# hezy18/SegMMInterest

Measured on AMD Instinct MI355X. Metric: train interactions/sec (segment-Transformer, B=512·S=40·D=768), higher is better.
Workload: dtype f32 (products via scaled fp16x2 split, 22-bit operands, fp32 accumulate; operands pre-split by their producers); 1 GPU; BASELINE config 2: synthetic SegMM B=512/GPU x S=40 x D_in=768 -> d=768, h=16, 2-layer segment encoder, image/image inputs, Lt=100 user tokens, interestBPR, dropout 0.1, AdamW; 8 distinct batches rotated; input=features; rows_per_gpu=512, global_batch=512, segments=40, feat_dim=768, in_dim=768, layers=2, parallelism=dp1, grad_allreduce_overlap=True, input_prefetch=False, delayed_scale_overflows=0, gemm_engine=f16x3p

## Files before the change

segmminterest_amd/csrc/capi.hip:

```cpp
#include <stdarg.h>
#include <stdio.h>
#include <string.h>
#include <stdlib.h>
#include <initializer_list>
#include <type_traits>

#include "../../include/segmm_hip.h"
#include "attention16.h"
#include "attention_pl.h"
#include "attention_stream.h"
#include "attention_wide.h"
#include "common.h"
#include "evalops.h"
#include "gemm.h"
#include "gemm_split.h"
#include "gemm_planes.h"
#include "gemm_planes8.h"
#include "gemm_planes4.h"
#include "loss.h"
#include "rowops.h"
#include "assemble.h"
#include "storeops.h"
#include "srops.h"

static int num_cus() {
    static int n = 0;
    if (n == 0) {
        int dev = 0;
        hipDeviceProp_t prop;
        if (hipGetDevice(&dev) == hipSuccess && hipGetDeviceProperties(&prop, dev) == hipSuccess) n = prop.multiProcessorCount;
        if (n <= 0) n = 256;
    }
    return n;
}
#ifdef SEGMM_STAMPS
static unsigned long long* g_segmm_stamps = nullptr;
extern "C" int segmm_debug_set_stamps(void* p) { g_segmm_stamps = (unsigned long long*)p; return 0; }
#endif

thread_local char g_segmm_err[512] = {0};

int segmm_fail(int code, const char* fmt, ...) {
    va_list ap;
    va_start(ap, fmt);
    vsnprintf(g_segmm_err, sizeof(g_segmm_err), fmt, ap);
    va_end(ap);
    return code;
}

#define LAUNCH_CHECK() SEGMM_CHECK_HIP(hipGetLastError())

StepState* g_segmm_step = nullptr;
static StepState* g_step_default = nullptr;
StepState* segmm_step_current() {
    if (g_segmm_step) return g_segmm_step;
    if (!g_step_default) {
        if (hipMalloc((void**)&g_step_default, sizeof(StepState)) != hipSuccess) return nullptr;
        (void)hipMemset(g_step_default, 0, sizeof(StepState));
    }
    return g_step_default;
}

using namespace segmm;

static inline int attn_keys_p(int La, int Lb) { return ((La + 15) & ~15) + ((Lb + 15) & ~15); }
static int attn_fill(AttnArgs& a, int B, int H, int dh, int Lq, int La, int Lb, const float* Qa, const float* Qb, int ldq,
                     const float* Ka, const float* Va, int ldka, const float* Kb, const float* Vb, int ldkb,
                     const uint8_t* mq, const uint8_t* mka, const uint8_t* mkb, float drop_p, uint64_t seed,
                     uint32_t site, bool planes_in = false) {
    SEGMM_REQUIRE(B > 0 && H > 0 && Lq > 0 && La >= 0 && Lb >= 0 && La + Lb > 0, "attn: empty dimension");
    if (La == 0) { Qa = Qb; Ka = Kb; Va = Vb; ldka = ldkb; mka = mkb; }
    if (Lb == 0) { Qb = Qa; Kb = Ka; Vb = Va; ldkb = ldka; mkb = mka; }
    SEGMM_REQUIRE(((Qa && Qb && Ka && Va && Kb && Vb) || (planes_in && !Qa && !Qb && !Ka && !Va && !Kb && !Vb)) && mq && mka && mkb, "attn: null pointer");
    SEGMM_REQUIRE(dh == 4 || dh == 8 || dh == 16 || dh == 32 || dh == 48 || dh == 64 || dh == 96 || dh == 128,
                  "attn: head dim %d not built (4,8,16,32,48,64,96,128)", dh);
    SEGMM_REQUIRE(!(planes_in && att_wide(dh)), "attn: input planes are not built for wide heads (head dim %d > 64): hand the fp32 views of Q / K / V", dh);
    SEGMM_REQUIRE(ldq % 4 == 0 && ldka % 4 == 0 && ldkb % 4 == 0, "attn: leading dims %% 4");
    SEGMM_REQUIRE(aligned16(Qa) && aligned16(Qb) && aligned16(Ka) && aligned16(Va) && aligned16(Kb) && aligned16(Vb), "attn: alignment");
    SEGMM_REQUIRE(Lq <= 256 && La <= 256 && Lb <= 256, "attn: Lq=%d, La=%d, Lb=%d not built (at most 256 queries and 256 keys per key block)", Lq, La, Lb);
    a.B = B; a.H = H; a.Lq = Lq; a.La = La; a.Lb = Lb;
    a.Qa = Qa; a.Qb = Qb; a.ldq = ldq; a.Ka = Ka; a.Va = Va; a.ldka = ldka; a.Kb = Kb; a.Vb = Vb; a.ldkb = ldkb;
    a.mq = mq; a.mka = mka; a.mkb = mkb;
    a.scale = 1.0f / sqrtf((float)dh);
    a.drop = make_drop(drop_p, seed, site);
    {
        const size_t ka = La ? ((size_t)B * La - 1) * ldka + (size_t)H * dh : 0, kb = Lb ? ((size_t)B * Lb - 1) * ldkb + (size_t)H * dh : 0;
        const size_t q = ((size_t)B * Lq - 1) * ldq + (size_t)H * dh;
        SEGMM_REQUIRE(((size_t)B * La + 16) * ldka * 4 < (1ull << 32) && ((size_t)B * Lb + 16) * ldkb * 4 < (1ull << 32) &&
                      ((size_t)B * Lq + 16) * ldq * 4 < (1ull << 32), "attn: a K/V/Q view exceeds the 4 GiB buffer-addressing window");
        a.ka_bytes = (uint32_t)(ka * 4); a.kb_bytes = (uint32_t)(kb * 4); a.q_bytes = (uint32_t)(q * 4);
    }
    return 0;
}

enum {
    K_ATTN, K_ATT_FWD_PL, K_ATT_FWD_LDS, K_ATT_FWD_KSPLIT, K_ATT_FWD_LDS_PAD, K_ATT_STREAM, K_ATT_FUSED_LAUNCH, K_ATT_MERGE, K_ATT_LDS_PAD, K_ATT_WAVES, K_ATT_WAVES_PL, K_ATT_REPAIR_WALK,
    K_ATT_HPB_FWD, K_ATT_HPB_DQ, K_ATT_HPB_DKV, K_L1NORM_REG, K_GEMM_BN, K_PL_VAR, K_PL_NJ, K_TN_VAR, K_LN_BWD_PARTS, K_DPRE_PLANES_ONLY, K_EMA_NT, K_LN_FWD_PARTS, K_COUNT
};
struct Knob { const char* name; int value; const char* doc; };
static Knob g_knobs[K_COUNT] = {
    {"ATTN", 1, "attention arithmetic: 0 (env: f32) exact-fp32 kernels only, 1 fp16x3 where measured faster, 2 (env: f16all) fp16x3 wherever built"},
    {"ATT_FWD_PL", 1, "planes-in forward when the caller hands input planes (0: never)"},
    {"ATT_FWD_LDS", 1, "LDS-DMA staged fp32 forward: 0 never, 1 heads with >= 4 query tiles, 2 wherever it fits"},
    {"ATT_FWD_KSPLIT", 1, "staged forward: key-tile groups per query tile"},
    {"ATT_FWD_LDS_PAD", 0, "probe: extra LDS bytes per forward workgroup (fewer workgroups per CU)"},
    {"ATT_STREAM", 0, "1: every fp32-view forward and every phase 0-3 backward through the streamed kernels (always taken above 192 padded keys)"},
    {"ATT_FUSED_LAUNCH", 2, "fused backward: 2 one launch per key block, 1 one launch for both"},
    {"ATT_MERGE", 1, "short heads: one workgroup per head for both key blocks in the fused backward"},
    {"ATT_LDS_PAD", 0, "probe: extra LDS bytes per backward workgroup"},
    {"ATT_WAVES", 4, "fused fp16x3 backward: waves per workgroup (key tiles in passes)"},
    {"ATT_WAVES_PL", 3, "planes-in fused backward: waves per workgroup, 1..4 (3: 40.7 KB of LDS -> four workgroups per CU for a 100-key block too)"},
    {"ATT_REPAIR_WALK", 512, "planes-in backward, repair launch: workgroups that walk the heads (0: one workgroup per head)"},
    {"ATT_HPB_FWD", 0, "forward workgroup shape heads | tiles << 8 (env: \"heads[,tiles]\"; 0: built-in)"},
    {"ATT_HPB_DQ", 0, "dQ kernel workgroup shape, as above"},
    {"ATT_HPB_DKV", 0, "dK/dV kernel workgroup shape, as above"},
    {"L1NORM_REG", 1, "L1 normalisation with the row held in registers"},
    {"GEMM_BN", 0, "on-the-fly GEMM: tile width override (0: built-in choice)"},
    {"PL_VAR", 4, "plane NT GEMM: 4 gemm_pl_nt4 (round 6: 128 x 256 tiles, two workgroups per CU) for K >= 768 and N >= 768, gemm_pl_nt8 otherwise; 44 gemm_pl_nt4 always; 8 gemm_pl_nt8 (round 3); 1: the round-2 fallback kernel for every launch"},
    {"PL_NJ", 0, "plane NT GEMM: tile width in 64-column units (0: modelled choice)"},
    {"TN_VAR", 8, "plane TN GEMM: 8 gemm_pl_tn4 (round 6: 128 x 256 tiles, two workgroups per CU) for few-tile and 128-row matrices, gemm_pl_tn8 (round 3) otherwise; 4 gemm_pl_tn4 wherever it fits; 88 gemm_pl_tn8 wherever it fits; 0: the round-2 fallback kernel for every launch"},
    {"LN_BWD_PARTS", 0, "LayerNorm backward: most workgroups (= partial rows of its column sums) per launch; 0: as many four-wave workgroups as are resident at the row width (768 at d = 768: one full round, no under-occupied tail)"},
    {"DPRE_PLANES_ONLY", 1, "embedding LayerNorm gradients as planes only + repair launch (no fp32 copy): 0 never, 1 for sites on the per-position grid today (rows * d >= 2^23), 2 wherever segmm_layernorm_bwd_pos_parts gives a grid (tests at small shapes), 3 as 1 for the user side only (A/B per site)"},
    {"EMA_NT", 0, "segmm_ema_update: 0 everything with the default cache policy, 1 the shadow loaded and stored nontemporally (p with the default policy); same bits (A/B: profiles/ema/)"},
    {"LN_FWD_PARTS", 0, "LayerNorm forward (d <= 1024): 0 one round of resident workgroups whose waves walk rows, grid by row width; 1 the one-wave-per-row form; 2 and up: that many workgroups in the walking form, clamped to 64..4096; same bits (A/B: profiles/row_stream/)"},
};
static bool g_knobs_ready = false;
static void knobs_init() {
    if (g_knobs_ready) return;
    g_knobs_ready = true;
    for (int k = 0; k < K_COUNT; ++k) {
        char name[64];
        snprintf(name, sizeof(name), "SEGMM_%s", g_knobs[k].name);
        const char* e = getenv(name);
        if (!e || !*e) continue;
        if (k == K_ATTN) g_knobs[k].value = !strcmp(e, "f32") ? 0 : !strcmp(e, "f16all") ? 2 : 1;
        else if (k == K_ATT_HPB_FWD || k == K_ATT_HPB_DQ || k == K_ATT_HPB_DKV) {
            const char* c = strchr(e, ',');
            g_knobs[k].value = (atoi(e) > 0 ? atoi(e) : 0) | ((c && atoi(c + 1) > 0 ? atoi(c + 1) : 0) << 8);
        } else g_knobs[k].value = atoi(e);
    }
}
static inline int knob(int k) { knobs_init(); return g_knobs[k].value; }
int segmm_config_set(const char* name, int value) {
    knobs_init();
    for (int k = 0; k < K_COUNT; ++k)
        if (!strcmp(name, g_knobs[k].name)) { const int prev = g_knobs[k].value; g_knobs[k].value = value; return prev; }
    return segmm_fail(-1, "segmm_config_set: no knob named %s (see segmm_config_dump)", name);
}
int segmm_config_dump(char* buf, int n) {
    knobs_init();
    int need = 0;
    for (int k = 0; k < K_COUNT; ++k) {
        char line[320];
        const int m = snprintf(line, sizeof(line), "SEGMM_%s=%d  # %s\n", g_knobs[k].name, g_knobs[k].value, g_knobs[k].doc);
        if (buf && need + m < n) memcpy(buf + need, line, (size_t)m + 1);
        need += m;
    }
    return need;
}

static int attn_f16() { return knob(K_ATTN); }

static void attn_shape(int n, int H, int max_waves, int want_default, int kn, int& wq, int& hpb) {
    wq = n;
    if (n > 5) {
        wq = 4;
        for (int w = 5; w >= 3; --w)
            if (n % w == 0) { wq = w; break; }
    }
    if (wq > max_waves) wq = max_waves;
    hpb = 1;
    const int e = knob(kn);
    int want = want_default;
    if (e & 0xff) {
        want = e & 0xff;
        if ((e >> 8) > 0 && (e >> 8) <= n && (e >> 8) <= max_waves) wq = e >> 8;
    }
    for (int c = want; c >= 1; --c)
        if (H % c == 0 && c * wq <= max_waves) { hpb = c; break; }
}

static bool attn_streamed(int Tp) { return Tp > 16 * 12 || knob(K_ATT_STREAM) != 0; }
template <class F>
static void attn_by_key_tiles(int Tp, F launch) {
    if (Tp <= 64) launch(std::integral_constant<int, 4>{});
    else if (Tp <= 160) launch(std::integral_constant<int, 10>{});
    else launch(std::integral_constant<int, 12>{});
}
template <int MAXW, class F>
static void attn_by_waves(int nw, F launch) {
    if (nw <= 4) launch(std::integral_constant<int, 4>{});
    else if (MAXW <= 8 || nw <= 8) launch(std::integral_constant<int, 8>{});
    else if constexpr (MAXW > 8) launch(std::integral_constant<int, 12>{});
}

template <int DH>
static bool attn_fwd_pl_takes(const AttnArgs& a) {
    if constexpr (DH % 16 != 0 || att_wide(DH)) return false;
    else {
        if (knob(K_ATT_FWD_PL) == 0) return false;
        const int nqt = (a.Lq + 15) / 16, T = a.La + a.Lb;
        return a.in.Qa && a.La % 4 == 0 && a.Lb % 4 == 0 && nqt <= ATT_PL_MAXW && T <= 16 * 12 &&
               attn_fwd_pl_lds_bytes<DH>(a.La, a.Lb) <= 160 * 1024 && (((uintptr_t)a.mka | (uintptr_t)a.mkb) & 3u) == 0;
    }
}
template <int DH>
static int attn_launch_fwd_pl(AttnArgs& a, hipStream_t s) {
// ... 297 lines not shown
#pragma unroll
    for (int i = 0; i < 8; ++i)
#pragma unroll
        for (int j = 0; j < 4; ++j) t += acc[i][j].x + acc[i][j].y + acc[i][j].z + acc[i][j].w;
    if (t == 12345.678f) out[0] = t;
}
}

namespace segmm {
__global__ void step_set_kernel(StepState* st, uint32_t lo, uint32_t hi, int step, float b1, float b2) {
    st->seed_lo = lo; st->seed_hi = hi; st->step = step;
    st->bc1 = step > 0 ? (float)(1.0 - pow((double)b1, (double)step)) : 1.f;
    st->bc2_sqrt = step > 0 ? (float)sqrt(1.0 - pow((double)b2, (double)step)) : 1.f;
    st->lr = (float)segmm_lr_at(*st, step - 1);
}
__global__ void step_advance_kernel(StepState* st, float b1, float b2) {
    const int t = st->step + 1;
    st->step = t;
    const uint32_t lo = mix32(st->seed_lo + 0x9E3779B9u * (uint32_t)t);
    st->seed_hi = mix32(st->seed_hi ^ lo ^ 0x85EBCA6Bu) & 0x7fffffffu;
    st->seed_lo = lo;
    st->bc1 = (float)(1.0 - pow((double)b1, (double)t));
    st->bc2_sqrt = (float)sqrt(1.0 - pow((double)b2, (double)t));
    st->lr = (float)segmm_lr_at(*st, t - 1);
}
__global__ void step_advance_guarded_kernel(StepState* st, float b1, float b2) {
    const int t = st->step + 1;
    st->step = t;
    const uint32_t lo = mix32(st->seed_lo + 0x9E3779B9u * (uint32_t)t);
    st->seed_hi = mix32(st->seed_hi ^ lo ^ 0x85EBCA6Bu) & 0x7fffffffu;
    st->seed_lo = lo;
    const int ta = t - (int)st->skipped;
    st->bc1 = ta > 0 ? (float)(1.0 - pow((double)b1, (double)ta)) : 1.f;
    st->bc2_sqrt = ta > 0 ? (float)sqrt(1.0 - pow((double)b2, (double)ta)) : 1.f;
    st->lr = (float)segmm_lr_at(*st, t - 1);
    st->skip = 0u;
}
__global__ void step_set_skipped_kernel(StepState* st, uint32_t skipped) {
    st->skip = 0u;
    st->skipped = skipped;
}
__global__ void step_schedule_kernel(StepState* st, int kind, float base_lr, int warmup_steps, float start_factor, int decay_steps,
                                     float eta_min, float gamma, int step_size) {
    st->kind = kind; st->base_lr = base_lr; st->warmup_steps = warmup_steps; st->start_factor = start_factor;
    st->decay_steps = decay_steps; st->eta_min = eta_min; st->gamma = gamma; st->step_size = step_size;
    st->lr = (float)segmm_lr_at(*st, st->step - 1);
}
__global__ void step_base_lr_kernel(StepState* st, float base_lr) {
    st->base_lr = base_lr;
    st->lr = (float)segmm_lr_at(*st, st->step - 1);
}
}

template <class F> static void with_bools(F&& f) { f(); }
template <class F, class... Bs> static void with_bools(F&& f, bool b, Bs... bs) {
    if (b) with_bools([&](auto... cs) { f(std::true_type{}, cs...); }, bs...);
    else with_bools([&](auto... cs) { f(std::false_type{}, cs...); }, bs...);
}

extern "C" {

const char* segmm_last_error(void) { return g_segmm_err; }
int segmm_abi_version(void) { return SEGMM_ABI_VERSION; }
int segmm_attn_mode(int mode) { const int prev = attn_f16(); if (mode >= 0 && mode <= 2) g_knobs[K_ATTN].value = mode; return prev; }

static PlaneOut plane_out(uint16_t* planes, int ld2, float* hdr, const float* scale_in) {
    PlaneOut po;
    po.p = (_Float16*)planes; po.ld2 = ld2; po.hdr = hdr; po.scale_in = scale_in;
    return po;
}
#define PLANE_OUT_CHECK(what, cols)                                                                                          \
    SEGMM_REQUIRE(!planes || (hdr && (cols) % 32 == 0 && ld2 % 64 == 0 && ld2 >= 2 * (cols) && aligned16(planes)),             \
                  what ": plane output needs a header, cols %% 32, ld2 %% 64, 16-byte alignment")

int segmm_l1norm(const float* x, float* y, float* inv_scale, int64_t rows, int D, float* amax, uint16_t* planes, int ld2, float* hdr,
                 const float* scale_in, segmm_stream_t stream) {
    PLANE_OUT_CHECK("l1norm", D);
    SEGMM_REQUIRE(x && (y || inv_scale || (planes && scale_in)), "l1norm: null pointer");
    SEGMM_REQUIRE(D > 0 && D % 4 == 0 && aligned16(x) && (!y || aligned16(y)), "l1norm: D %% 4 / alignment (D=%d)", D);
    if (rows <= 0) return 0;
    const int wpb = 4;
    const int reg_form = knob(K_L1NORM_REG);
    const dim3 grid((unsigned)((rows + wpb - 1) / wpb)), block(64 * wpb);
#define L1R(V) hipLaunchKernelGGL((l1norm_reg_kernel<V>), grid, block, 0, (hipStream_t)stream, x, y, inv_scale, (long long)rows, D, amax, plane_out(planes, ld2, hdr, scale_in))
    if (reg_form && D <= 256) L1R(1);
    else if (reg_form && D <= 512) L1R(2);
    else if (reg_form && D <= 768) L1R(3);
    else if (reg_form && D <= 1024) L1R(4);
    else if (reg_form && D <= 1536) L1R(6);
    else if (reg_form && D <= 2048) L1R(8);
    else hipLaunchKernelGGL(l1norm_kernel, grid, block, 0, (hipStream_t)stream, x, y, inv_scale, (long long)rows, D, amax, plane_out(planes, ld2, hdr, scale_in));
#undef L1R
    LAUNCH_CHECK();
    return 0;
}

static inline bool aligned8(const void* p) { return (((uintptr_t)p) & 7u) == 0; }
#define ROW_H_LAUNCH(KERNEL, ...)                                                                                        \
    do {                                                                                                                 \
        if (elem == SEGMM_ELEM_F16) { ROW_H_LAUNCH_V(KERNEL, ELEM_F16, __VA_ARGS__); }                                   \
        else { ROW_H_LAUNCH_V(KERNEL, ELEM_BF16, __VA_ARGS__); }                                                         \
    } while (0)
#define ROW_H_LAUNCH_V(KERNEL, E, ...)                                                                                   \
    do {                                                                                                                 \
        if (D <= 256) hipLaunchKernelGGL((KERNEL<E, 1>), grid, block, 0, (hipStream_t)stream, __VA_ARGS__);              \
        else if (D <= 512) hipLaunchKernelGGL((KERNEL<E, 2>), grid, block, 0, (hipStream_t)stream, __VA_ARGS__);         \
        else if (D <= 768) hipLaunchKernelGGL((KERNEL<E, 3>), grid, block, 0, (hipStream_t)stream, __VA_ARGS__);         \
        else if (D <= 1024) hipLaunchKernelGGL((KERNEL<E, 4>), grid, block, 0, (hipStream_t)stream, __VA_ARGS__);        \
        else if (D <= 1536) hipLaunchKernelGGL((KERNEL<E, 6>), grid, block, 0, (hipStream_t)stream, __VA_ARGS__);        \
        else if (D <= 256 * ROW_MAXV) hipLaunchKernelGGL((KERNEL<E, 8>), grid, block, 0, (hipStream_t)stream, __VA_ARGS__); \
        else hipLaunchKernelGGL((KERNEL<E, 0>), grid, block, 0, (hipStream_t)stream, __VA_ARGS__);                       \
    } while (0)

int segmm_l1norm_h(const uint16_t* x, int elem, float* y, float* inv_scale, int64_t rows, int D, float* amax, uint16_t* planes, int ld2,
                   float* hdr, const float* scale_in, segmm_stream_t stream) {
    PLANE_OUT_CHECK("l1norm_h", D);
    SEGMM_REQUIRE(elem == SEGMM_ELEM_F16 || elem == SEGMM_ELEM_BF16, "l1norm_h: elem = %d (SEGMM_ELEM_F16 = 1, SEGMM_ELEM_BF16 = 2)", elem);
    SEGMM_REQUIRE(x && (y || inv_scale || (planes && scale_in)), "l1norm_h: null pointer");
    SEGMM_REQUIRE(D > 0 && D % 4 == 0 && aligned8(x) && (!y || aligned16(y)), "l1norm_h: D %% 4 / alignment (D=%d)", D);
    if (rows <= 0) return 0;
    const dim3 grid((unsigned)((rows + 3) / 4)), block(256);
    ROW_H_LAUNCH(l1norm_h_kernel, x, y, inv_scale, (long long)rows, D, amax, plane_out(planes, ld2, hdr, scale_in));
    LAUNCH_CHECK();
    return 0;
}

static inline bool aligned4(const void* p) { return (((uintptr_t)p) & 3u) == 0; }
static inline bool elem8(int elem) { return elem == SEGMM_ELEM_E4M3 || elem == SEGMM_ELEM_E5M2 || elem == SEGMM_ELEM_I8; }
#define ROW_B_LAUNCH(KERNEL, ...)                                                                                        \
    do {                                                                                                                 \
        if (elem == SEGMM_ELEM_E4M3) { ROW_H_LAUNCH_V(KERNEL, ELEM_E4M3, __VA_ARGS__); }                                 \
        else if (elem == SEGMM_ELEM_E5M2) { ROW_H_LAUNCH_V(KERNEL, ELEM_E5M2, __VA_ARGS__); }                            \
        else { ROW_H_LAUNCH_V(KERNEL, ELEM_I8, __VA_ARGS__); }                                                           \
    } while (0)

int segmm_l1norm_b(const uint8_t* x, int elem, float* y, float* inv_scale, int64_t rows, int D, float* amax, uint16_t* planes, int ld2,
                   float* hdr, const float* scale_in, segmm_stream_t stream) {
    PLANE_OUT_CHECK("l1norm_b", D);
    SEGMM_REQUIRE(elem8(elem), "l1norm_b: elem = %d (SEGMM_ELEM_E4M3 = 3, SEGMM_ELEM_E5M2 = 4, SEGMM_ELEM_I8 = 5)", elem);
    SEGMM_REQUIRE(x && (y || inv_scale || (planes && scale_in)), "l1norm_b: null pointer");
    SEGMM_REQUIRE(D > 0 && D % 4 == 0 && aligned4(x) && (!y || aligned16(y)), "l1norm_b: D %% 4 / alignment (D=%d)", D);
    if (rows <= 0) return 0;
    const dim3 grid((unsigned)((rows + 3) / 4)), block(256);
    ROW_B_LAUNCH(l1norm_b_kernel, x, y, inv_scale, (long long)rows, D, amax, plane_out(planes, ld2, hdr, scale_in));
    LAUNCH_CHECK();
    return 0;
}

int segmm_quantize_rows(const float* x, int64_t rows, int D, int elem, uint8_t* q, float* scale_out, segmm_stream_t stream) {
    SEGMM_REQUIRE(elem8(elem), "quantize_rows: elem = %d (SEGMM_ELEM_E4M3 = 3, SEGMM_ELEM_E5M2 = 4, SEGMM_ELEM_I8 = 5)", elem);
    SEGMM_REQUIRE(x && q && rows >= 0, "quantize_rows: null pointer / rows");
    SEGMM_REQUIRE(D > 0 && D % 4 == 0 && aligned16(x) && aligned4(q) && (!scale_out || aligned4(scale_out)),
                  "quantize_rows: D %% 4 / alignment (D=%d)", D);
    if (rows <= 0) return 0;
    const dim3 grid((unsigned)((rows + 3) / 4)), block(256);
    if (elem == SEGMM_ELEM_E4M3) hipLaunchKernelGGL((quantize_rows_kernel<ELEM_E4M3>), grid, block, 0, (hipStream_t)stream, x, (long long)rows, D, q, scale_out);
    else if (elem == SEGMM_ELEM_E5M2) hipLaunchKernelGGL((quantize_rows_kernel<ELEM_E5M2>), grid, block, 0, (hipStream_t)stream, x, (long long)rows, D, q, scale_out);
    else hipLaunchKernelGGL((quantize_rows_kernel<ELEM_I8>), grid, block, 0, (hipStream_t)stream, x, (long long)rows, D, q, scale_out);
    LAUNCH_CHECK();
    return 0;
}

static int gemm_impl(int layout, int M, int N, int K, const float* A, int lda, const float* B, int ldb, float* C, int ldc,
                     const float* bias, const float* row_scale, const float* residual, int ldr, int res_period,
                     int activation, float* aux, int ldaux, float drop_p, uint64_t seed, uint32_t site, int splits,
                     float* workspace, int accumulate, int engine, const uint16_t* a_planes, long long a_pstride,
                     const uint16_t* b_planes, long long b_pstride, int nplanes, const float* a_amax, int a_namax,
// ... 1941 lines not shown
```

segmminterest_amd/csrc/gemm_planes.h:

```cpp
#pragma once
#include <type_traits>
#include "gemm_split.h"

namespace segmm {

struct PlaneOperand {
    const _Float16* p; int ld2;
    uint32_t bytes;
    const float* hdr;
    const float* f32; int ldf;
};
struct PGemmX {
    PlaneOperand A, B;
    _Float16* Cp; int ldc2; float* c_hdr;
    const float* c_scale_in;
    int write_c;
    int repair;
    float* colsum_out; float* colsum_ws;
    int dbg;
    unsigned long long* stamps;
};

#ifdef SEGMM_GEMM_PROBE
#define SEGMM_GEMM_DBG(q) ((q).dbg)
// ... 448 lines not shown
    if (do_colsum) k_loop(std::true_type{});
    else k_loop(std::false_type{});

    const bool split = gridDim.z > 1;
    if (do_colsum && (lane & 31) == 0) {
        float* dst = split ? q.colsum_ws + (size_t)kz * p.M : q.colsum_out;
        const float inv_a = 1.f / sa;
#pragma unroll
        for (int r = 0; r < 16; ++r) {
            const int m = m0 + wm * 128 + wn * 32 + (r & 3) + 8 * (r >> 2) + 4 * (lane >> 5);
            if (m < p.M) dst[m] = (!split && p.residual) ? dst[m] + accb[r] * inv_a : accb[r] * inv_a;
        }
    }
    float* Cs = (float*)smem + wave * (32 * 64);
    const float inv_ab = (1.f / sa) * (1.f / sb);
    float* Cout = split ? p.C + (size_t)kz * (size_t)p.slab_stride : p.C;
    float am = 0.f;
#pragma unroll 1
    for (int i = 0; i < 4; ++i) {
        f32x16 c[2];
        switch (i) {
            case 0: c[0] = acc[0][0]; c[1] = acc[0][1]; break;
            case 1: c[0] = acc[1][0]; c[1] = acc[1][1]; break;
            case 2: c[0] = acc[2][0]; c[1] = acc[2][1]; break;
            default: c[0] = acc[3][0]; c[1] = acc[3][1]; break;
        }
        epi_strip_write<2>(c, Cs, lane);
        if (split) epi_strip_emit<true, 2>(p, q, Cs, lane, m0 + wm * 128 + i * 32, n0 + wn * 64, inv_ab, 0.f, Cout, am);
        else epi_strip_emit<false, 2>(p, q, Cs, lane, m0 + wm * 128 + i * 32, n0 + wn * 64, inv_ab, 0.f, Cout, am);
    }
}

__global__ __launch_bounds__(256) void split_p32_kernel(const float* __restrict__ x, long long rows, int cols, int ld,
                                                        _Float16* __restrict__ planes, int ld2, float* hdr, int mode) {
    __shared__ float red[8];
    float s;
    if (mode == 0) s = site_exact_scale(hdr, red, threadIdx.x, 256);
    else s = hdr[0];
    const int c4n = cols >> 2;
    const long long n4 = rows * c4n;
    float am = 0.f;
    bool nan = false;
    for (long long i = blockIdx.x * (long long)blockDim.x + threadIdx.x; i < n4; i += (long long)gridDim.x * blockDim.x) {
        const long long r = i / c4n;
        const int c = (int)(i - r * c4n) << 2;
        const f32x4 v = *(const f32x4*)(x + r * ld + c);
        plane_store4_pair(planes, ld2, r, c, v, s);
        am = absmax4(am, v);
        nan |= (v.x != v.x) | (v.y != v.y) | (v.z != v.z) | (v.w != v.w);
    }
    if (mode == 0) {
        if (blockIdx.x == 0 && threadIdx.x == 0) { hdr[0] = s; hdr[1] = 0.f; }
    } else {
        site_commit(hdr, am, blockIdx.x * 4 + (threadIdx.x >> 6), s);
        if (nan && s > 0.f) ((volatile unsigned int*)hdr)[1] = 1u;
    }
}
__global__ __launch_bounds__(256) void split_p32_transpose_kernel(const float* __restrict__ x, int R, int Cc, int ld,
                                                                  _Float16* __restrict__ planes, int ld2, const float* hdr) {
    __shared__ float tile[32][33];
    const float s = hdr[0];
    const int r0 = blockIdx.y * 32, c0 = blockIdx.x * 32;
    const int tx = threadIdx.x & 31, ty = threadIdx.x >> 5;
#pragma unroll
    for (int k = 0; k < 4; ++k) {
        const int r = r0 + ty + 8 * k, c = c0 + tx;
        tile[ty + 8 * k][tx] = (r < R && c < Cc) ? x[(size_t)r * ld + c] : 0.f;
    }
    __syncthreads();
#pragma unroll
    for (int k = 0; k < 4; ++k) {
        const int c = c0 + ty + 8 * k, r = r0 + tx;
        if (c < Cc && r < R) {
            const float v = tile[tx][ty + 8 * k];
            const _Float16 h = (_Float16)__builtin_fmaf(v, s, 0.f);
            const _Float16 l = (_Float16)__builtin_fmaf(v, s, -(float)h);
            _Float16* o = planes + (size_t)c * ld2 + ((r >> 5) << 6) + (r & 31);
            o[0] = h; o[32] = l;
        }
    }
}

struct WMat { long long off; int R, Cc, tr, tile0, tcols; };
__global__ __launch_bounds__(256) void wabsmax_kernel(const float* __restrict__ flat, const WMat* __restrict__ desc, float* hdr) {
    const WMat m = desc[blockIdx.y];
    const float* x = flat + m.off;
    const long long n4 = (long long)m.R * m.Cc / 4;
    float am = 0.f;
    for (long long i = blockIdx.x * (long long)blockDim.x + threadIdx.x; i < n4; i += (long long)gridDim.x * blockDim.x)
        am = absmax4(am, *(const f32x4*)(x + 4 * i));
    am = wave_max(am);
    if ((threadIdx.x & 63) == 0) hdr[(size_t)blockIdx.y * SITE_FLOATS + SITE_HDR + blockIdx.x * 4 + (threadIdx.x >> 6)] = am;
}
__global__ __launch_bounds__(256) void wsplit_kernel(const float* __restrict__ flat, const WMat* __restrict__ desc, int n_mats, float* hdr,
                                                     _Float16* __restrict__ wpl, _Float16* __restrict__ wTpl) {
    __shared__ float tile[32][33];
    __shared__ float red[8];
    int mi = 0;
    while (mi + 1 < n_mats && (int)blockIdx.x >= desc[mi + 1].tile0) ++mi;
    const WMat m = desc[mi];
    float* h = hdr + (size_t)mi * SITE_FLOATS;
    const float s = site_exact_scale(h, red, threadIdx.x, 256);
    const int t = blockIdx.x - m.tile0;
    const int r0 = (t / m.tcols) * 32, c0 = (t % m.tcols) * 32;
    if (t == 0 && threadIdx.x == 0) { h[0] = s; h[1] = 0.f; }
    const float* x = flat + m.off;
    const int tx = threadIdx.x & 31, ty = threadIdx.x >> 5;
#pragma unroll
    for (int k = 0; k < 4; ++k) {
        const int r = r0 + ty + 8 * k, c = c0 + tx;
        const float v = (r < m.R && c < m.Cc) ? x[(size_t)r * m.Cc + c] : 0.f;
        tile[ty + 8 * k][tx] = v;
        if (r < m.R && c < m.Cc) {
            const _Float16 hi = (_Float16)__builtin_fmaf(v, s, 0.f);
            const _Float16 lo = (_Float16)__builtin_fmaf(v, s, -(float)hi);
            _Float16* o = wpl + 2 * m.off + (size_t)r * (2 * m.Cc) + ((c >> 5) << 6) + (c & 31);
            o[0] = hi; o[32] = lo;
        }
    }
    if (!m.tr) return;
    __syncthreads();
#pragma unroll
    for (int k = 0; k < 4; ++k) {
        const int c = c0 + ty + 8 * k, r = r0 + tx;
        if (c < m.Cc && r < m.R) {
            const float v = tile[tx][ty + 8 * k];
            const _Float16 hi = (_Float16)__builtin_fmaf(v, s, 0.f);
            const _Float16 lo = (_Float16)__builtin_fmaf(v, s, -(float)hi);
            _Float16* o = wTpl + 2 * m.off + (size_t)c * (2 * m.R) + ((r >> 5) << 6) + (r & 31);
            o[0] = hi; o[32] = lo;
        }
    }
}

}
```

segmminterest_amd/csrc/rowops.h:

```cpp
#pragma once
#include "common.h"

namespace segmm {
constexpr int ROW_MAXV = 8;

__global__ __launch_bounds__(256) void l1norm_kernel(const float* __restrict__ x, float* y, float* inv_scale, long long rows, int D,
                                                     float* amax, PlaneOut po) {
    const int lane = threadIdx.x & 63;
    const long long row = (long long)blockIdx.x * (blockDim.x >> 6) + (threadIdx.x >> 6);
    if (row >= rows) return;
    const float* xr = x + row * D;
    float s = 0.f;
    for (int c = lane * 4; c < D; c += 256) {
        const f32x4 v = *(const f32x4*)(xr + c);
        s += fabsf(v.x) + fabsf(v.y) + fabsf(v.z) + fabsf(v.w);
    }
    s = wave_sum(s);
    const float inv = 1.0f / (s + 1e-6f);
    if (inv_scale && lane == 0) inv_scale[row] = inv;
    const float ps = plane_scale(po);
    if (y || ps > 0.f) {
        const float den = s + 1e-6f;
        float am = 0.f;
        for (int c = lane * 4; c < D; c += 256) {
            f32x4 v = *(const f32x4*)(xr + c);
            v.x /= den; v.y /= den; v.z /= den; v.w /= den;
            if (y) *(f32x4*)(y + row * D + c) = v;
            if (ps > 0.f) plane_store4_pair(po.p, po.ld2, row, c, v, ps);
            am = absmax4(am, v);
        }
        plane_finish(po, amax, am, (unsigned)row, ps, row == 0 && lane == 0);
    }
}

template <int V>
__global__ __launch_bounds__(256) void l1norm_reg_kernel(const float* __restrict__ x, float* y, float* inv_scale, long long rows, int D,
                                                         float* amax, PlaneOut po) {
    const int lane = threadIdx.x & 63;
    const long long row = (long long)blockIdx.x * (blockDim.x >> 6) + (threadIdx.x >> 6);
    if (row >= rows) return;
    const float* xr = x + row * D;
    f32x4 v[V];
    float s = 0.f;
#pragma unroll
    for (int i = 0; i < V; ++i) {
        const int c = lane * 4 + i * 256;
        v[i] = f32x4{0.f, 0.f, 0.f, 0.f};
        if (c < D) { v[i] = ld_row4b(xr + c); s += fabsf(v[i].x) + fabsf(v[i].y) + fabsf(v[i].z) + fabsf(v[i].w); }
    }
    s = wave_sum(s);
    const float inv = 1.0f / (s + 1e-6f);
    if (inv_scale && lane == 0) inv_scale[row] = inv;
    const float ps = plane_scale(po);
    if (y || ps > 0.f) {
        const float den = s + 1e-6f;
        float am = 0.f;
#pragma unroll
        for (int i = 0; i < V; ++i) {
            const int c = lane * 4 + i * 256;
            if (c < D) {
                f32x4 o = v[i];
                o.x /= den; o.y /= den; o.z /= den; o.w /= den;
                if (y) st_row4b(y + row * D + c, o);
                if (ps > 0.f) plane_store4_pair(po.p, po.ld2, row, c, o, ps);
                am = absmax4(am, o);
            }
        }
        plane_finish(po, amax, am, (unsigned)row, ps, row == 0 && lane == 0);
    }
}

template <int ELEM, int V>
__global__ __launch_bounds__(256) void l1norm_h_kernel(const uint16_t* __restrict__ x, float* y, float* inv_scale, long long rows, int D,
                                                       float* amax, PlaneOut po) {
    const int lane = threadIdx.x & 63;
    const long long row = (long long)blockIdx.x * (blockDim.x >> 6) + (threadIdx.x >> 6);
    if (row >= rows) return;
    const uint16_t* xr = x + row * D;
    uint32_t ra[V > 0 ? V : 1], rb[V > 0 ? V : 1];
    float s = 0.f;
    if constexpr (V > 0) {
#pragma unroll
        for (int i = 0; i < V; ++i) {
            const int c = lane * 4 + i * 256;
            ra[i] = rb[i] = 0u;
            if (c < D) {
                const u32x2 w = ld_row4h(xr + c);
                ra[i] = w.x; rb[i] = w.y;
                const f32x4 v = widen4<ELEM>(ra[i], rb[i]);
                s += fabsf(v.x) + fabsf(v.y) + fabsf(v.z) + fabsf(v.w);
            }
        }
    } else {
        for (int c = lane * 4; c < D; c += 256) {
            const f32x4 v = widen4<ELEM>(ld_row4h(xr + c));
            s += fabsf(v.x) + fabsf(v.y) + fabsf(v.z) + fabsf(v.w);
        }
    }
    s = wave_sum(s);
    const float inv = 1.0f / (s + 1e-6f);
    if (inv_scale && lane == 0) inv_scale[row] = inv;
    const float ps = plane_scale(po);
    if (y || ps > 0.f) {
        const float den = s + 1e-6f;
        float am = 0.f;
        if constexpr (V > 0) {
#pragma unroll
            for (int i = 0; i < V; ++i) {
                const int c = lane * 4 + i * 256;
                if (c < D) {
                    f32x4 o = widen4<ELEM>(ra[i], rb[i]);
                    o.x /= den; o.y /= den; o.z /= den; o.w /= den;
                    if (y) st_row4b(y + row * D + c, o);
                    if (ps > 0.f) plane_store4_pair(po.p, po.ld2, row, c, o, ps);
                    am = absmax4(am, o);
                }
            }
        } else {
            for (int c = lane * 4; c < D; c += 256) {
                f32x4 o = widen4<ELEM>(ld_row4h(xr + c));
                o.x /= den; o.y /= den; o.z /= den; o.w /= den;
                if (y) *(f32x4*)(y + row * D + c) = o;
                if (ps > 0.f) plane_store4_pair(po.p, po.ld2, row, c, o, ps);
                am = absmax4(am, o);
            }
        }
        plane_finish(po, amax, am, (unsigned)row, ps, row == 0 && lane == 0);
    }
}

template <int ELEM, int V>
__global__ __launch_bounds__(256) void l1norm_b_kernel(const uint8_t* __restrict__ x, float* y, float* inv_scale, long long rows, int D,
                                                       float* amax, PlaneOut po) {
    const int lane = threadIdx.x & 63;
    const long long row = (long long)blockIdx.x * (blockDim.x >> 6) + (threadIdx.x >> 6);
    if (row >= rows) return;
    const uint8_t* xr = x + row * D;
    uint32_t rw[V > 0 ? V : 1];
    float s = 0.f;
    if constexpr (V > 0) {
#pragma unroll
        for (int i = 0; i < V; ++i) {
            const int c = lane * 4 + i * 256;
            rw[i] = 0u;
            if (c < D) {
                rw[i] = ld_row4q(xr + c);
                const f32x4 v = widen4<ELEM>(rw[i]);
                s += fabsf(v.x) + fabsf(v.y) + fabsf(v.z) + fabsf(v.w);
            }
        }
    } else {
        for (int c = lane * 4; c < D; c += 256) {
// ... 1129 lines not shown
```

Baseline: 145,300 interactions/s.

## Persistent row-walking L1 norm, batched weight absmax loads, vectorized weight split

```diff
diff --git a/segmminterest_amd/csrc/capi.hip b/segmminterest_amd/csrc/capi.hip
--- a/segmminterest_amd/csrc/capi.hip
+++ b/segmminterest_amd/csrc/capi.hip
@@ -95,7 +95,7 @@
 
 enum {
     K_ATTN, K_ATT_FWD_PL, K_ATT_FWD_LDS, K_ATT_FWD_KSPLIT, K_ATT_FWD_LDS_PAD, K_ATT_STREAM, K_ATT_FUSED_LAUNCH, K_ATT_MERGE, K_ATT_LDS_PAD, K_ATT_WAVES, K_ATT_WAVES_PL, K_ATT_REPAIR_WALK,
-    K_ATT_HPB_FWD, K_ATT_HPB_DQ, K_ATT_HPB_DKV, K_L1NORM_REG, K_GEMM_BN, K_PL_VAR, K_PL_NJ, K_TN_VAR, K_LN_BWD_PARTS, K_DPRE_PLANES_ONLY, K_EMA_NT, K_LN_FWD_PARTS, K_COUNT
+    K_ATT_HPB_FWD, K_ATT_HPB_DQ, K_ATT_HPB_DKV, K_L1NORM_REG, K_GEMM_BN, K_PL_VAR, K_PL_NJ, K_TN_VAR, K_LN_BWD_PARTS, K_DPRE_PLANES_ONLY, K_EMA_NT, K_LN_FWD_PARTS, K_L1NORM_PARTS, K_COUNT
 };
 struct Knob { const char* name; int value; const char* doc; };
 static Knob g_knobs[K_COUNT] = {
@@ -123,6 +123,7 @@
     {"DPRE_PLANES_ONLY", 1, "embedding LayerNorm gradients as planes only + repair launch (no fp32 copy): 0 never, 1 for sites on the per-position grid today (rows * d >= 2^23), 2 wherever segmm_layernorm_bwd_pos_parts gives a grid (tests at small shapes), 3 as 1 for the user side only (A/B per site)"},
     {"EMA_NT", 0, "segmm_ema_update: 0 everything with the default cache policy, 1 the shadow loaded and stored nontemporally (p with the default policy); same bits (A/B: profiles/ema/)"},
     {"LN_FWD_PARTS", 0, "LayerNorm forward (d <= 1024): 0 one round of resident workgroups whose waves walk rows, grid by row width; 1 the one-wave-per-row form; 2 and up: that many workgroups in the walking form, clamped to 64..4096; same bits (A/B: profiles/row_stream/)"},
+    {"L1NORM_PARTS", 0, "L1 normalisation of float32 rows in registers that commits maxima (amax or planes): 0 one round of resident workgroups whose waves walk rows and commit once; 1 one wave per row, a commit per row; 2 and up: that many workgroups, clamped to 64..4096; same bits (A/B: profiles/plane_stores/)"},
 };
 static bool g_knobs_ready = false;
 static void knobs_init() {
@@ -586,7 +587,13 @@
     const int wpb = 4;
     const int reg_form = knob(K_L1NORM_REG);
     const dim3 grid((unsigned)((rows + wpb - 1) / wpb)), block(64 * wpb);
-#define L1R(V) hipLaunchKernelGGL((l1norm_reg_kernel<V>), grid, block, 0, (hipStream_t)stream, x, y, inv_scale, (long long)rows, D, amax, plane_out(planes, ld2, hdr, scale_in))
+    dim3 rgrid = grid;
+    if (amax || planes) {
+        const int k = knob(K_L1NORM_PARTS);
+        const unsigned cap = k == 1 ? 0u : k >= 2 ? (unsigned)(k < 64 ? 64 : k > 4096 ? 4096 : k) : D <= 768 ? 2048u : D <= 1024 ? 1536u : D <= 1536 ? 1280u : 1024u;
+        if (cap && rgrid.x > cap) rgrid.x = cap;
+    }
+#define L1R(V) hipLaunchKernelGGL((l1norm_reg_kernel<V>), rgrid, block, 0, (hipStream_t)stream, x, y, inv_scale, (long long)rows, D, amax, plane_out(planes, ld2, hdr, scale_in))
     if (reg_form && D <= 256) L1R(1);
     else if (reg_form && D <= 512) L1R(2);
     else if (reg_form && D <= 768) L1R(3);
diff --git a/segmminterest_amd/csrc/gemm_planes.h b/segmminterest_amd/csrc/gemm_planes.h
--- a/segmminterest_amd/csrc/gemm_planes.h
+++ b/segmminterest_amd/csrc/gemm_planes.h
@@ -554,16 +554,32 @@
 }
 
 struct WMat { long long off; int R, Cc, tr, tile0, tcols; };
+constexpr int WABSMAX_INFLIGHT = 8;
 __global__ __launch_bounds__(256) void wabsmax_kernel(const float* __restrict__ flat, const WMat* __restrict__ desc, float* hdr) {
     const WMat m = desc[blockIdx.y];
     const float* x = flat + m.off;
     const long long n4 = (long long)m.R * m.Cc / 4;
     float am = 0.f;
-    for (long long i = blockIdx.x * (long long)blockDim.x + threadIdx.x; i < n4; i += (long long)gridDim.x * blockDim.x)
-        am = absmax4(am, *(const f32x4*)(x + 4 * i));
+    const long long step = (long long)gridDim.x * blockDim.x;
+    long long i = blockIdx.x * (long long)blockDim.x + threadIdx.x;
+    for (; i + (WABSMAX_INFLIGHT - 1) * step < n4; i += WABSMAX_INFLIGHT * step) {
+        f32x4 v[WABSMAX_INFLIGHT];
+#pragma unroll
+        for (int k = 0; k < WABSMAX_INFLIGHT; ++k) v[k] = *(const f32x4*)(x + 4 * (i + k * step));
+#pragma unroll
+        for (int k = 0; k < WABSMAX_INFLIGHT; ++k) am = absmax4(am, v[k]);
+    }
+    for (; i < n4; i += step) am = absmax4(am, *(const f32x4*)(x + 4 * i));
     am = wave_max(am);
     if ((threadIdx.x & 63) == 0) hdr[(size_t)blockIdx.y * SITE_FLOATS + SITE_HDR + blockIdx.x * 4 + (threadIdx.x >> 6)] = am;
 }
+struct WTerm { uint16_t hi, lo; };
+__device__ __forceinline__ WTerm wsplit_term(float v, float s) {
+    const _Float16 hi = (_Float16)__builtin_fmaf(v, s, 0.f);
+    const _Float16 lo = (_Float16)__builtin_fmaf(v, s, -(float)hi);
+    return {__builtin_bit_cast(uint16_t, hi), __builtin_bit_cast(uint16_t, lo)};
+}
+__device__ __forceinline__ uint32_t pack_h2(uint16_t a, uint16_t b) { return (uint32_t)a | ((uint32_t)b << 16); }
 __global__ __launch_bounds__(256) void wsplit_kernel(const float* __restrict__ flat, const WMat* __restrict__ desc, int n_mats, float* hdr,
                                                      _Float16* __restrict__ wpl, _Float16* __restrict__ wTpl) {
     __shared__ float tile[32][33];
@@ -577,32 +593,38 @@
     const int r0 = (t / m.tcols) * 32, c0 = (t % m.tcols) * 32;
     if (t == 0 && threadIdx.x == 0) { h[0] = s; h[1] = 0.f; }
     const float* x = flat + m.off;
-    const int tx = threadIdx.x & 31, ty = threadIdx.x >> 5;
+    const int ty = threadIdx.x >> 3, q = threadIdx.x & 7;
+    f32x4 v = {0.f, 0.f, 0.f, 0.f};
+    if (r0 + ty < m.R) v = *(const f32x4*)(x + (size_t)(r0 + ty) * m.Cc + c0 + 4 * q);
+    tile[ty][4 * q] = v.x; tile[ty][4 * q + 1] = v.y; tile[ty][4 * q + 2] = v.z; tile[ty][4 * q + 3] = v.w;
+    __syncthreads();
+    const int k8 = (q & 3) * 8;
+    const bool lo = q >= 4;
+    auto terms8 = [&](bool down) {
+        uint16_t e[8];
+#pragma unroll
+        for (int j = 0; j < 8; ++j) {
+            const WTerm w = wsplit_term(down ? tile[k8 + j][ty] : tile[ty][k8 + j], s);
+            e[j] = lo ? w.lo : w.hi;
+        }
+        return make_uint4(pack_h2(e[0], e[1]), pack_h2(e[2], e[3]), pack_h2(e[4], e[5]), pack_h2(e[6], e[7]));
+    };
+    if (r0 + ty < m.R) *(uint4*)(wpl + 2 * m.off + (size_t)(r0 + ty) * (2 * m.Cc) + 2 * c0 + (lo ? 32 : 0) + k8) = terms8(false);
+    if (!m.tr) return;
+    if ((m.R & 31) == 0) {
+        *(uint4*)(wTpl + 2 * m.off + (size_t)(c0 + ty) * (2 * m.R) + 2 * r0 + (lo ? 32 : 0) + k8) = terms8(true);
+        return;
+    }
+    const int tx = threadIdx.x & 31, tz = threadIdx.x >> 5;
 #pragma unroll
     for (int k = 0; k < 4; ++k) {
-        const int r = r0 + ty + 8 * k, c = c0 + tx;
-        const float v = (r < m.R && c < m.Cc) ? x[(size_t)r * m.Cc + c] : 0.f;
-        tile[ty + 8 * k][tx] = v;
-        if (r < m.R && c < m.Cc) {
-            const _Float16 hi = (_Float16)__builtin_fmaf(v, s, 0.f);
-            const _Float16 lo = (_Float16)__builtin_fmaf(v, s, -(float)hi);
-            _Float16* o = wpl + 2 * m.off + (size_t)r * (2 * m.Cc) + ((c >> 5) << 6) + (c & 31);
-            o[0] = hi; o[32] = lo;
-        }
-    }
-    if (!m.tr) return;
-    __syncthreads();
-#pragma unroll
-    for (int k = 0; k < 4; ++k) {
-        const int c = c0 + ty + 8 * k, r = r0 + tx;
-        if (c < m.Cc && r < m.R) {
-            const float v = tile[tx][ty + 8 * k];
-            const _Float16 hi = (_Float16)__builtin_fmaf(v, s, 0.f);
-            const _Float16 lo = (_Float16)__builtin_fmaf(v, s, -(float)hi);
-            _Float16* o = wTpl + 2 * m.off + (size_t)c * (2 * m.R) + ((r >> 5) << 6) + (r & 31);
-            o[0] = hi; o[32] = lo;
-        }
-    }
-}
-
-}
+        const int c = c0 + tz + 8 * k, rr = r0 + tx;
+        if (rr < m.R) {
+            const WTerm w = wsplit_term(tile[tx][tz + 8 * k], s);
+            uint16_t* o = (uint16_t*)wTpl + 2 * m.off + (size_t)c * (2 * m.R) + ((rr >> 5) << 6) + (rr & 31);
+            o[0] = w.hi; o[32] = w.lo;
+        }
+    }
+}
+
+}
diff --git a/segmminterest_amd/csrc/rowops.h b/segmminterest_amd/csrc/rowops.h
--- a/segmminterest_amd/csrc/rowops.h
+++ b/segmminterest_amd/csrc/rowops.h
@@ -37,37 +37,57 @@
 __global__ __launch_bounds__(256) void l1norm_reg_kernel(const float* __restrict__ x, float* y, float* inv_scale, long long rows, int D,
                                                          float* amax, PlaneOut po) {
     const int lane = threadIdx.x & 63;
-    const long long row = (long long)blockIdx.x * (blockDim.x >> 6) + (threadIdx.x >> 6);
+    const long long stride = (long long)gridDim.x * (blockDim.x >> 6);
+    long long row = (long long)blockIdx.x * (blockDim.x >> 6) + (threadIdx.x >> 6);
     if (row >= rows) return;
-    const float* xr = x + row * D;
-    f32x4 v[V];
-    float s = 0.f;
+    f32x4 nx[V];
 #pragma unroll
     for (int i = 0; i < V; ++i) {
         const int c = lane * 4 + i * 256;
-        v[i] = f32x4{0.f, 0.f, 0.f, 0.f};
-        if (c < D) { v[i] = ld_row4b(xr + c); s += fabsf(v[i].x) + fabsf(v[i].y) + fabsf(v[i].z) + fabsf(v[i].w); }
-    }
-    s = wave_sum(s);
-    const float inv = 1.0f / (s + 1e-6f);
-    if (inv_scale && lane == 0) inv_scale[row] = inv;
+        nx[i] = f32x4{0.f, 0.f, 0.f, 0.f};
+        if (c < D) nx[i] = ld_row4b(x + row * D + c);
+    }
     const float ps = plane_scale(po);
-    if (y || ps > 0.f) {
-        const float den = s + 1e-6f;
-        float am = 0.f;
+    const bool one_slot = (stride & (AMAX_SLOTS - 1)) == 0 || row + stride >= rows;
+    const long long row0 = row;
+    float am = 0.f;
+    for (; row < rows; row += stride) {
+        f32x4 v[V];
+        float s = 0.f;
 #pragma unroll
         for (int i = 0; i < V; ++i) {
             const int c = lane * 4 + i * 256;
-            if (c < D) {
-                f32x4 o = v[i];
-                o.x /= den; o.y /= den; o.z /= den; o.w /= den;
-                if (y) st_row4b(y + row * D + c, o);
-                if (ps > 0.f) plane_store4_pair(po.p, po.ld2, row, c, o, ps);
-                am = absmax4(am, o);
-            }
-        }
-        plane_finish(po, amax, am, (unsigned)row, ps, row == 0 && lane == 0);
-    }
+            v[i] = nx[i];
+            if (c < D) s += fabsf(v[i].x) + fabsf(v[i].y) + fabsf(v[i].z) + fabsf(v[i].w);
+        }
+        if (row + stride < rows) {
+#pragma unroll
+            for (int i = 0; i < V; ++i) {
+                const int c = lane * 4 + i * 256;
+                if (c < D) nx[i] = ld_row4b(x + (row + stride) * D + c);
+            }
+        }
+        s = wave_sum(s);
+        const float inv = 1.0f / (s + 1e-6f);
+        if (inv_scale && lane == 0) inv_scale[row] = inv;
+        if (y || ps > 0.f) {
+            const float den = s + 1e-6f;
+            if (!one_slot) am = 0.f;
+#pragma unroll
+            for (int i = 0; i < V; ++i) {
+                const int c = lane * 4 + i * 256;
+                if (c < D) {
+                    f32x4 o = v[i];
+                    o.x /= den; o.y /= den; o.z /= den; o.w /= den;
+                    if (y) st_row4b(y + row * D + c, o);
+                    if (ps > 0.f) plane_store4_pair(po.p, po.ld2, row, c, o, ps);
+                    am = absmax4(am, o);
+                }
+            }
+            if (!one_slot) plane_finish(po, amax, am, (unsigned)row, ps, row == 0 && lane == 0);
+        }
+    }
+    if (one_slot && (y || ps > 0.f)) plane_finish(po, amax, am, (unsigned)row0, ps, row0 == 0 && lane == 0);
 }
 
 template <int ELEM, int V>
```

Result: no change. 146,200 interactions/s (median of 3 runs) (+0.6%).
